# chihyaoma/cyclical-visual-captioning

Hardware: AMD Instinct MI355X
Metric: caption decode-steps/sec (BxT) at N=100,D=2048 (higher is better)
Workload: dtype f32; 1 GPU; cfg2: greedy caption decode; B_per_gpu=64, N=100, F=480, D=2048, A=1024, E=1024, V=5000, T=20, beam=1, hip_graph=True, parallelism=clips sharded over 1 rank(s), no collective, schedule=embedding-gate table (att-LSTM GEMM over K = 2R + one table row per word)

## Files before the change

### cyclical-visual-captioning_amd/build_hip.py

```python
#!/usr/bin/env python3
from __future__ import annotations

import glob
import os
import subprocess
import sys

HERE = os.path.dirname(os.path.abspath(__file__))
CSRC = os.path.join(HERE, "csrc")
OUT_DIR = os.path.join(HERE, "cvc", "lib")
OUT = os.path.join(OUT_DIR, "libcvc_hip.so")
HIPCC = os.environ.get("HIPCC", "/opt/rocm/bin/hipcc")


EXPERIMENTAL_SOURCES = ("gemm_gsk.hip", "gemm_packed_ks.hip")


def experimental() -> bool:
    return os.environ.get("CVC_EXPERIMENTAL", "0") not in ("", "0")


def sources():
    return [f for f in sorted(glob.glob(os.path.join(CSRC, "*.hip")))
            if experimental() or os.path.basename(f) not in EXPERIMENTAL_SOURCES]


def deps():
    inc = os.path.join(os.path.dirname(HERE), "include")
    return sources() + sorted(glob.glob(os.path.join(CSRC, "*.h"))) + \
        [os.path.join(inc, h) for h in ("cvc_hip.h", "cvc_hip_blocks.h", "cvc_hip_experimental.h")]


def source_hash() -> str:
    import hashlib
    h = hashlib.sha256()
    for f in sorted(deps(), key=os.path.basename):
        h.update(os.path.basename(f).encode() + b"\0")
        h.update(open(f, "rb").read())
    return h.hexdigest()[:16]


STAMP = os.path.join(OUT_DIR, "libcvc_hip.flags")


def extra_flags() -> str:
    return " ".join(os.environ.get("CVC_EXTRA_HIPCC_FLAGS", "").split() + (["-DCVC_EXPERIMENTAL"] if experimental() else []))


def up_to_date() -> bool:
    if not os.path.exists(OUT):
        return False
    built_with = open(STAMP).read().strip() if os.path.exists(STAMP) else ""
    if built_with != extra_flags():
        return False
    t = os.path.getmtime(OUT)
    return all(os.path.getmtime(f) <= t for f in deps())


NO_SCRATCH_KERNELS = {"gemm_nn.hip": ("skinny_gemm_nn_split128_kernel",), "gemm_packed.hip": ("skinny_gemm_packed_kernel",)}


def check_no_scratch(src: str, remarks: str):
    import re
    want = NO_SCRATCH_KERNELS.get(os.path.basename(src), ())
    seen = set()
    for block in remarks.split("remark: Function Name: ")[1:]:
        name = block.split()[0]
        hit = next((k for k in want if k in name), None)
        if hit is None:
            continue
        seen.add(hit)
        vals = {k: int(v) for k, v in re.findall(r"remark:\s+(ScratchSize \[bytes/lane\]|SGPRs Spill|VGPRs Spill): (\d+)", block)}
        bad = {k: v for k, v in vals.items() if v != 0}
        if bad or len(vals) < 3:
            raise RuntimeError(f"{os.path.basename(src)}: kernel {name} must not use scratch or spill (inline-assembly loads in "
                               f"flight): {vals}")
    missing = set(want) - seen
    if missing:
        raise RuntimeError(f"{os.path.basename(src)}: no resource-usage remark for {sorted(missing)} (renamed kernel?)")


def build(force: bool = False, verbose: bool = True) -> str:
    if not force and up_to_date():
        return OUT
    os.makedirs(OUT_DIR, exist_ok=True)
    objs = []
    obj_dir = os.path.join(HERE, "build")
    os.makedirs(obj_dir, exist_ok=True)
    procs = []
    for src in sources():
        obj = os.path.join(obj_dir, os.path.basename(src) + ".o")
        objs.append(obj)
        cmd = [HIPCC, "--offload-arch=gfx950", "-O3", "-std=c++17", "-fPIC", "-fvisibility=hidden", "-Wno-comment", "-c", src, "-o", obj]
        cmd += extra_flags().split()
        checked = os.path.basename(src) in NO_SCRATCH_KERNELS
        if checked:
            cmd.append("-Rpass-analysis=kernel-resource-usage")
        if verbose:
            print(" ".join(cmd), flush=True)
        procs.append((cmd, src, checked, subprocess.Popen(cmd, stderr=subprocess.PIPE if checked else None, text=checked or None)))
    for cmd, src, checked, p in procs:
        err = p.communicate()[1] if checked else None
        if p.wait() != 0:
            if err:
                sys.stderr.write("\n".join(l for l in err.splitlines() if "kernel-resource-usage" not in l)[-8000:] + "\n")
            raise RuntimeError("hipcc failed: " + " ".join(cmd))
        if checked:
            check_no_scratch(src, err)
    objs = [o for o in objs if os.path.exists(o)]
    cmd = [HIPCC, "--offload-arch=gfx950", "-shared", "-fPIC", "-o", OUT] + objs + ["-ldl"]
    if verbose:
        print(" ".join(cmd), flush=True)
    subprocess.check_call(cmd)
    with open(STAMP, "w") as f:
        f.write(extra_flags() + "\n")
    return OUT


if __name__ == "__main__":
    print(build(force="--force" in sys.argv))
```

### cyclical-visual-captioning_amd/csrc/attn_scores.h

```cpp
#pragma once
#include "cvc_common.h"
#ifdef CVC_EXPERIMENTAL
#include "gsk.h"
#endif
#include <stdlib.h>
#include <type_traits>

namespace {

#ifndef CVC_SCORE_ROWS
#define CVC_SCORE_ROWS 32
#endif
constexpr int ROWS_PER_WG = CVC_SCORE_ROWS;
constexpr int ROWS_PER_WG_MAX = 128;
constexpr int SCORE_WG = 256;

struct ScoreArgs {
    cvc_attn_set set[2];
    int chunks0;
    const float* q;
    const float* q_bias;
    int q_nparts;
    long long q_part_stride;
    long long q_ld;
    const float* w_a;
    const float* b_a;
    float inv_temp;
    int nq, A;
    int nq_total, q0;
    int rows_per_wg;
#ifdef CVC_EXPERIMENTAL
    int q_from_slab;
    GskSegs q_slab;
#endif
};

template <int NPL>
__device__ __forceinline__ f32x4 sum_planes_fixed(const float* src, long long stride) {
    f32x4 pv[NPL];
#pragma unroll
    for (int p = 0; p < NPL; ++p) pv[p] = ld4(src + (size_t)p * stride);
    f32x4 v = pv[0];
#pragma unroll
    for (int p = 1; p < NPL; ++p) v += pv[p];
    return v;
}
__device__ __forceinline__ f32x4 sum_planes(const float* src, int n, long long stride) {
    switch (n) {
        case 1: return ld4(src);
        case 2: return sum_planes_fixed<2>(src, stride);
        case 4: return sum_planes_fixed<4>(src, stride);
        case 8: return sum_planes_fixed<8>(src, stride);
        case 16: return sum_planes_fixed<16>(src, stride);
        default: break;
    }
    f32x4 v = ld4(src);
    for (int p = 1; p < n; ++p) v += ld4(src + (size_t)p * stride);
    return v;
}

template <int KIND, int NCH, int QG>
__global__ __launch_bounds__(SCORE_WG) void attn_scores_kernel(ScoreArgs a) {
    constexpr bool FACTORABLE = KIND == CVC_ATTN_ADDITIVE && QG > 1;
    extern __shared__ __attribute__((aligned(16))) float smem[];
    const int nq_pad = (a.nq + QG - 1) / QG * QG;
    float* q_s = smem;
    float* w_s = smem + (size_t)nq_pad * a.A;
    constexpr float EXP_C = 2.8853900817779268f;
    const int clip = blockIdx.y;
    const int s = (int)blockIdx.x < a.chunks0 ? 0 : 1;
    const int chunk = s == 0 ? blockIdx.x : blockIdx.x - a.chunks0;
    const cvc_attn_set& S = a.set[s];
    const int A = a.A, nq = a.nq, n = S.n;
    const int tid = threadIdx.x, lane = tid & 63, wave = tid >> 6;
    const float fill = (S.stream & 4) ? -__builtin_inff() : CVC_MIN_VALUE;
    const float bias_a = (KIND == CVC_ATTN_ADDITIVE && a.b_a != nullptr) ? a.b_a[0] : 0.f;

    int q_big = 0;
    for (int i = tid * 4; i < nq_pad * A; i += SCORE_WG * 4) {
        f32x4 v = {0, 0, 0, 0};
#ifdef CVC_EXPERIMENTAL
        if (i < nq * A && a.q_from_slab) {
            const int col = i % A, row = clip * a.nq_total + a.q0 + i / A, blk = col >> 5;
            const int nseg = gsk_nseg(a.q_slab, blk >> 3);
            const float* src = gsk_part(a.q_slab, blk >> 3, 0, blk & 7) + (size_t)row * 32 + (col & 31);
            v = ld4(src);
            for (int p = 1; p < nseg; ++p) v += ld4(src + (size_t)p * (8 * 2048));
            if (a.q_bias != nullptr) v += ld4(a.q_bias + col);
        } else
#endif
        if (i < nq * A) {
            const float* src = a.q + ((size_t)clip * a.nq_total + a.q0 + i / A) * a.q_ld + i % A;
            v = sum_planes(src, a.q_nparts, a.q_part_stride);
            if (a.q_bias != nullptr) v += ld4(a.q_bias + (i % A));
        }
        if (KIND == CVC_ATTN_ADDITIVE) v *= EXP_C;
        if constexpr (FACTORABLE)
            q_big |= !(fabsf(v.x) <= 30.f && fabsf(v.y) <= 30.f && fabsf(v.z) <= 30.f && fabsf(v.w) <= 30.f);
        st4(q_s + i, v);
    }
    if (KIND == CVC_ATTN_ADDITIVE)
        for (int i = tid * 4; i < A; i += SCORE_WG * 4) st4(w_s + i, ld4(a.w_a + i));
    bool factored = false;
    if constexpr (FACTORABLE) {
#ifndef CVC_SCORE_NO_FACTORED
        factored = __syncthreads_or(q_big) == 0;
#else
        __syncthreads();
#endif
        if (factored) {
            for (int i = tid * 4; i < nq_pad * A; i += SCORE_WG * 4) {
                f32x4 v = ld4(q_s + i);
                v.x = __builtin_amdgcn_exp2f(v.x); v.y = __builtin_amdgcn_exp2f(v.y);
                v.z = __builtin_amdgcn_exp2f(v.z); v.w = __builtin_amdgcn_exp2f(v.w);
                st4(q_s + i, v);
            }
            for (int i = tid * 4; i < A; i += SCORE_WG * 4) st4(w_s + i, ld4(w_s + i) * -2.0f);
            __syncthreads();
        }
    } else {
        __syncthreads();
    }

    const int row0 = chunk * a.rows_per_wg;
    const int row_end = min(n, row0 + a.rows_per_wg);
    const float* P = S.proj + (size_t)clip * n * A;

    auto emit = [&](float sc, int q0, int r, bool masked) __attribute__((always_inline)) {
        if (lane < QG && q0 + lane < nq) {
            if (masked) sc = fill;
            const size_t o = ((size_t)clip * a.nq_total + a.q0 + q0 + lane) * n + r;
            S.scores[o] = sc;
            if (S.frame_masked != nullptr)
                S.frame_masked[o] = S.frame_mask[o] != 0 ? fill : sc;
        }
    };
    auto rows = [&](auto stream_tag, auto fact_tag, auto exact_tag) __attribute__((always_inline)) {
        constexpr bool STREAM = decltype(stream_tag)::value;
        constexpr bool FACT = decltype(fact_tag)::value;
        constexpr bool EXACT = decltype(exact_tag)::value;
        const int A = EXACT ? NCH * 256 : a.A;
#define LDF(ptr) (STREAM ? __builtin_nontemporal_load(reinterpret_cast<const f32x4*>(ptr)) : ld4(ptr))
    f32x4 cur[NCH], nxt[NCH];
    int colc[NCH];
    bool cok[NCH];
#pragma unroll
    for (int j = 0; j < NCH; ++j) {
        const int col = (j * 64 + lane) * 4;
        cok[j] = EXACT || col < A;
        colc[j] = cok[j] ? col : A - 4;
    }
    int r = row0 + wave;
    if (r >= row_end) return;
    unsigned mbits = 0;
    if (S.mask != nullptr) {
        const int rr = r + 4 * lane;
        const bool m = rr < row_end && S.mask[(size_t)clip * n + (rr < row_end ? rr : r)] != 0;
        mbits = (unsigned)__builtin_amdgcn_ballot_w64(m);
    }
    float w_total = 0.f;
    if constexpr (FACT) {
#pragma unroll
        for (int j = 0; j < NCH; ++j) {
            const f32x4 w4 = ld4(w_s + colc[j]);
            if (cok[j]) w_total += (w4.x + w4.y) + (w4.z + w4.w);
        }
        w_total = -0.5f * wave_sum(w_total);
    }
#pragma unroll
    for (int j = 0; j < NCH; ++j) cur[j] = LDF(P + (size_t)r * A + colc[j]);
    auto step = [&](f32x4 (&cur)[NCH], f32x4 (&nxt)[NCH], int r, int k) __attribute__((always_inline)) {
#if defined(CVC_SC_ABL) && CVC_SC_ABL == 2
        const int rn = r;
#else
        const int rn = min(r + 4, row_end - 1);
#endif
#pragma unroll
        for (int j = 0; j < NCH; ++j) nxt[j] = LDF(P + (size_t)rn * A + colc[j]);
        const bool masked = (mbits >> k) & 1u;
        if constexpr (FACT) {
            using f32x2 = __attribute__((ext_vector_type(2))) float;
            f32x4 ep[NCH], w2[NCH];
#pragma unroll
            for (int j = 0; j < NCH; ++j) {
                const f32x4 x = cur[j] * EXP_C;
                ep[j].x = __builtin_amdgcn_exp2f(__builtin_amdgcn_fmed3f(x.x, -62.f, 62.f));
                ep[j].y = __builtin_amdgcn_exp2f(__builtin_amdgcn_fmed3f(x.y, -62.f, 62.f));
                ep[j].z = __builtin_amdgcn_exp2f(__builtin_amdgcn_fmed3f(x.z, -62.f, 62.f));
                ep[j].w = __builtin_amdgcn_exp2f(__builtin_amdgcn_fmed3f(x.w, -62.f, 62.f));
                w2[j] = cok[j] ? ld4(w_s + colc[j]) : f32x4{0, 0, 0, 0};
            }
            for (int q0 = 0; q0 < nq; q0 += QG) {
                f32x2 acc2[QG];
                float acc[QG];
#pragma unroll
                for (int u = 0; u < QG; ++u) acc2[u] = f32x2{0.f, 0.f};
#pragma unroll
                for (int j = 0; j < NCH; ++j) {
#pragma unroll
                    for (int u = 0; u < QG; ++u) {
                        const f32x4 eq = ld4(q_s + (q0 + u) * A + colc[j]);
                        const f32x2 d01 = __builtin_elementwise_fma(f32x2{ep[j].x, ep[j].y}, f32x2{eq.x, eq.y}, f32x2{1.0f, 1.0f});
                        const f32x2 d23 = __builtin_elementwise_fma(f32x2{ep[j].z, ep[j].w}, f32x2{eq.z, eq.w}, f32x2{1.0f, 1.0f});
                        const f32x2 r01 = {fast_rcp(d01.x), fast_rcp(d01.y)}, r23 = {fast_rcp(d23.x), fast_rcp(d23.y)};
                        acc2[u] = __builtin_elementwise_fma(f32x2{w2[j].x, w2[j].y}, r01, acc2[u]);
                        acc2[u] = __builtin_elementwise_fma(f32x2{w2[j].z, w2[j].w}, r23, acc2[u]);
                    }
                }
#pragma unroll
                for (int u = 0; u < QG; ++u) acc[u] = (w_total + wave_sum(acc2[u].x + acc2[u].y)) + bias_a;
                float sc = acc[0];
#pragma unroll
                for (int u = 1; u < QG; ++u) sc = lane == u ? acc[u] : sc;
                emit(sc, q0, r, masked);
            }
        } else
        for (int q0 = 0; q0 < nq; q0 += QG) {
            float acc[QG];
            using f32x2 = __attribute__((ext_vector_type(2))) float;
            f32x2 acc2[QG];
#pragma unroll
            for (int u = 0; u < QG; ++u) { acc[u] = 0.f; acc2[u] = f32x2{0.f, 0.f}; }
#pragma unroll
            for (int j = 0; j < NCH; ++j) {
                f32x4 p = cok[j] ? cur[j] : f32x4{0, 0, 0, 0};
                f32x4 w4 = {0, 0, 0, 0};
                if (KIND == CVC_ATTN_ADDITIVE) {
                    w4 = ld4(w_s + colc[j]);
                    if (!cok[j]) w4 = f32x4{0, 0, 0, 0};
                    p *= EXP_C;
                }
#pragma unroll
                for (int u = 0; u < QG; ++u) {
                    const f32x4 q4 = ld4(q_s + (q0 + u) * A + colc[j]);
                    if (KIND == CVC_ATTN_ADDITIVE) {
                        const f32x4 x = p + q4;
                        if constexpr (QG > 1) {
                            const f32x2 e01 = {__builtin_amdgcn_exp2f(x.x), __builtin_amdgcn_exp2f(x.y)};
                            const f32x2 e23 = {__builtin_amdgcn_exp2f(x.z), __builtin_amdgcn_exp2f(x.w)};
                            const f32x2 d01 = e01 + 1.0f, d23 = e23 + 1.0f;
                            const f32x2 r01 = {fast_rcp(d01.x), fast_rcp(d01.y)}, r23 = {fast_rcp(d23.x), fast_rcp(d23.y)};
                            const f32x2 t01 = __builtin_elementwise_fma(f32x2{-2.0f, -2.0f}, r01, f32x2{1.0f, 1.0f});
                            const f32x2 t23 = __builtin_elementwise_fma(f32x2{-2.0f, -2.0f}, r23, f32x2{1.0f, 1.0f});
                            acc2[u] = __builtin_elementwise_fma(f32x2{w4.x, w4.y}, t01, acc2[u]);
                            acc2[u] = __builtin_elementwise_fma(f32x2{w4.z, w4.w}, t23, acc2[u]);
                        } else {
                            acc[u] = fmaf(w4.x, fmaf(-2.0f, fast_rcp(1.0f + __builtin_amdgcn_exp2f(x.x)), 1.0f), acc[u]);
                            acc[u] = fmaf(w4.y, fmaf(-2.0f, fast_rcp(1.0f + __builtin_amdgcn_exp2f(x.y)), 1.0f), acc[u]);
                            acc[u] = fmaf(w4.z, fmaf(-2.0f, fast_rcp(1.0f + __builtin_amdgcn_exp2f(x.z)), 1.0f), acc[u]);
                            acc[u] = fmaf(w4.w, fmaf(-2.0f, fast_rcp(1.0f + __builtin_amdgcn_exp2f(x.w)), 1.0f), acc[u]);
                        }
                    } else {
                        acc[u] += p.x * q4.x + p.y * q4.y + p.z * q4.z + p.w * q4.w;
                    }
                }
            }
            if constexpr (KIND == CVC_ATTN_ADDITIVE && QG > 1) {
#pragma unroll
                for (int u = 0; u < QG; ++u) acc[u] = acc2[u].x + acc2[u].y;
            }
#pragma unroll
            for (int u = 0; u < QG; ++u) acc[u] = KIND == CVC_ATTN_ADDITIVE ? wave_sum(acc[u]) + bias_a : wave_sum(acc[u]) * a.inv_temp;
            float sc = acc[0];
#pragma unroll
            for (int u = 1; u < QG; ++u) sc = lane == u ? acc[u] : sc;
            emit(sc, q0, r, masked);
        }
    };
    for (int k = 0;;) {
        step(cur, nxt, r, k);
        r += 4; ++k;
        if (r >= row_end) break;
        step(nxt, cur, r, k);
        r += 4; ++k;
        if (r >= row_end) break;
    }
#undef LDF
    };
    using T_ = std::true_type;
    using F_ = std::false_type;
    if constexpr (FACTORABLE) {
        if (factored) {
            if (a.A == NCH * 256) { if (S.stream & 1) rows(T_{}, T_{}, T_{}); else rows(F_{}, T_{}, T_{}); }
            else { if (S.stream & 1) rows(T_{}, T_{}, F_{}); else rows(F_{}, T_{}, F_{}); }
            return;
        }
    }
    if (S.stream & 1) rows(T_{}, F_{}, F_{}); else rows(F_{}, F_{}, F_{});
}

template <int KIND, int QG>
int launch_scores_q(const ScoreArgs& a, dim3 grid, size_t lds, hipStream_t st) {
    const int nch = (a.A + 255) / 256;
#define CVC_SC(N) hipLaunchKernelGGL((attn_scores_kernel<KIND, N, QG>), grid, dim3(SCORE_WG), lds, st, a)
    if (nch <= 1) CVC_SC(1);
    else if (nch <= 2) CVC_SC(2);
    else if (nch <= 4) CVC_SC(4);
    else if (nch <= 8) CVC_SC(8);
    else if (nch <= 16) CVC_SC(16);
    else return CVC_E_TOOBIG;
#undef CVC_SC
    return cvc_launch_status();
}

inline int score_group(int nq) {
    if (nq <= 1) return 1;
    const int p4 = (nq + 3) / 4 * 4, p5 = (nq + 4) / 5 * 5;
    return p5 <= p4 ? 5 : 4;
}

template <int KIND>
int launch_scores(const ScoreArgs& a, dim3 grid, size_t lds, hipStream_t st) {
    switch (score_group(a.nq)) {
        case 1: return launch_scores_q<KIND, 1>(a, grid, lds, st);
        case 4: return launch_scores_q<KIND, 4>(a, grid, lds, st);
        default: return launch_scores_q<KIND, 5>(a, grid, lds, st);
    }
}


inline int score_rows_per_wg(int nclip, int n0, int n1, size_t lds_bytes) {
    static const int forced = [] { const char* e = getenv("CVC_SCORE_ROWS_RT"); return e ? atoi(e) : 0; }();
    if (forced >= 4 && forced <= ROWS_PER_WG_MAX) return forced;
    int per_cu = (int)((160 * 1024) / (lds_bytes > 0 ? lds_bytes : 1));
    per_cu = per_cu > 4 ? 4 : (per_cu < 1 ? 1 : per_cu);
    const long long slots = 256LL * per_cu;
    int best = ROWS_PER_WG;
    double best_cost = 1e30;
    for (int r = 8; r <= ROWS_PER_WG_MAX; ++r) {
        const long long wgs = (long long)nclip * ((n0 + r - 1) / r + (n1 > 0 ? (n1 + r - 1) / r : 0));
        const long long rounds = (wgs + slots - 1) / slots;
        const double cost = (double)rounds * ((r + 3) / 4 + 1.5);
        if (cost < best_cost - 1e-9) { best_cost = cost; best = r; }
    }
    return best;
}

inline int run_scores(int kind, const float* q, const float* w_a, const float* b_a, float inv_temp,
                      const cvc_attn_set* sets, int nsets, int nclip, int nq, int A, hipStream_t st,
                      int q_nparts = 1, const float* q_bias = nullptr, const void* q_slab = nullptr, long long q_ld = 0,
                      long long q_part_stride = 0) {
    int q_per_launch = (int)((64 * 1024) / ((size_t)A * 4)) - 1;
    if (q_per_launch < 1) return CVC_E_TOOBIG;
    if (q_per_launch > nq) q_per_launch = nq;
    if (q_per_launch < nq && q_per_launch >= 5) q_per_launch = q_per_launch / 5 * 5;
    while (q_per_launch > 1 && (size_t)((q_per_launch + score_group(q_per_launch) - 1) / score_group(q_per_launch) *
                                        score_group(q_per_launch) + 1) * A * 4 > 64 * 1024) --q_per_launch;
    ScoreArgs sa;
    sa.set[0] = sets[0];
    sa.set[1] = nsets > 1 ? sets[1] : sets[0];
    sa.q = q; sa.w_a = w_a; sa.b_a = b_a; sa.inv_temp = inv_temp; sa.A = A; sa.nq_total = nq;
    sa.q_nparts = q_nparts < 1 ? 1 : q_nparts; sa.q_bias = q_bias;
    sa.q_ld = q_ld > 0 ? q_ld : A;
    sa.q_part_stride = q_part_stride > 0 ? q_part_stride : (long long)nclip * nq * A;
#ifdef CVC_EXPERIMENTAL
    sa.q_from_slab = q_slab != nullptr;
    sa.q_slab = q_slab != nullptr ? *static_cast<const GskSegs*>(q_slab) : GskSegs{};
#else
    if (q_slab != nullptr) return CVC_E_BADARG;
#endif
    for (int q0 = 0; q0 < nq; q0 += q_per_launch) {
        sa.q0 = q0;
        sa.nq = nq - q0 < q_per_launch ? nq - q0 : q_per_launch;
        const int qg = score_group(sa.nq);
        const size_t lds1 = (size_t)((sa.nq + qg - 1) / qg * qg + 1) * A * sizeof(float);
        sa.rows_per_wg = sa.nq > 1 ? score_rows_per_wg(nclip, sets[0].n, nsets > 1 ? sets[1].n : 0, lds1) : ROWS_PER_WG;
        sa.chunks0 = (sets[0].n + sa.rows_per_wg - 1) / sa.rows_per_wg;
        const int chunks1 = nsets > 1 ? (sets[1].n + sa.rows_per_wg - 1) / sa.rows_per_wg : 0;
        dim3 g1(sa.chunks0 + chunks1, nclip);
        int rc = kind == CVC_ATTN_ADDITIVE ? launch_scores<CVC_ATTN_ADDITIVE>(sa, g1, lds1, st)
                                           : launch_scores<CVC_ATTN_DOT>(sa, g1, lds1, st);
        if (rc != 0) return rc;
    }
    return 0;
}

}
```

Baseline: 330,800 decode-steps/s.

## Balance single-query attention score work across CUs with row shares and prefetch

For the single-query (decode) path, the score kernel now splits the combined rows of both attention sets into evenly sized shares whose count is chosen from the CU count and clip count, so one workgroup may span both sets. Each wave prefetches its first projection row and mask before the query-plane summation, the 16-plane query sum is split into two batches of loads, and launch bounds request higher occupancy for small-NCH QG=1 variants. The build adds a scratch/spill check for those kernels. This aims to cut tail imbalance and load latency in the per-step attention, at the cost of more register pressure and extra code paths.

```diff
diff --git a/cyclical-visual-captioning_amd/build_hip.py b/cyclical-visual-captioning_amd/build_hip.py
--- a/cyclical-visual-captioning_amd/build_hip.py
+++ b/cyclical-visual-captioning_amd/build_hip.py
@@ -57,7 +57,8 @@
     return all(os.path.getmtime(f) <= t for f in deps())
 
 
-NO_SCRATCH_KERNELS = {"gemm_nn.hip": ("skinny_gemm_nn_split128_kernel",), "gemm_packed.hip": ("skinny_gemm_packed_kernel",)}
+NO_SCRATCH_KERNELS = {"gemm_nn.hip": ("skinny_gemm_nn_split128_kernel",), "gemm_packed.hip": ("skinny_gemm_packed_kernel",),
+                      "attn_fwd.hip": ("attn_scores_kernelILi0ELi4ELi1E", "attn_scores_kernelILi1ELi4ELi1E")}
 
 
 def check_no_scratch(src: str, remarks: str):
diff --git a/cyclical-visual-captioning_amd/csrc/attn_scores.h b/cyclical-visual-captioning_amd/csrc/attn_scores.h
--- a/cyclical-visual-captioning_amd/csrc/attn_scores.h
+++ b/cyclical-visual-captioning_amd/csrc/attn_scores.h
@@ -29,6 +29,8 @@
     int nq, A;
     int nq_total, q0;
     int rows_per_wg;
+    int shares;
+    int rows_total;
 #ifdef CVC_EXPERIMENTAL
     int q_from_slab;
     GskSegs q_slab;
@@ -59,8 +61,10 @@
     return v;
 }
 
+constexpr int score_min_waves(int nch, int qg) { return qg == 1 && nch <= 4 ? 5 : 1; }
+
 template <int KIND, int NCH, int QG>
-__global__ __launch_bounds__(SCORE_WG) void attn_scores_kernel(ScoreArgs a) {
+__global__ __launch_bounds__(SCORE_WG, score_min_waves(NCH, QG)) void attn_scores_kernel(ScoreArgs a) {
     constexpr bool FACTORABLE = KIND == CVC_ATTN_ADDITIVE && QG > 1;
     extern __shared__ __attribute__((aligned(16))) float smem[];
     const int nq_pad = (a.nq + QG - 1) / QG * QG;
@@ -68,13 +72,53 @@
     float* w_s = smem + (size_t)nq_pad * a.A;
     constexpr float EXP_C = 2.8853900817779268f;
     const int clip = blockIdx.y;
-    const int s = (int)blockIdx.x < a.chunks0 ? 0 : 1;
-    const int chunk = s == 0 ? blockIdx.x : blockIdx.x - a.chunks0;
-    const cvc_attn_set& S = a.set[s];
-    const int A = a.A, nq = a.nq, n = S.n;
+    const int A = a.A, nq = a.nq;
     const int tid = threadIdx.x, lane = tid & 63, wave = tid >> 6;
-    const float fill = (S.stream & 4) ? -__builtin_inff() : CVC_MIN_VALUE;
+    int part_set[2], part_lo[2], part_hi[2], nparts = 1;
+    if (QG == 1 && a.shares > 0) {
+        const int n0 = a.set[0].n;
+        const int lo = (int)((long long)blockIdx.x * a.rows_total / a.shares);
+        const int hi = (int)((long long)(blockIdx.x + 1) * a.rows_total / a.shares);
+        if (lo < n0) {
+            part_set[0] = 0; part_lo[0] = lo; part_hi[0] = min(hi, n0);
+            part_set[1] = 1; part_lo[1] = 0; part_hi[1] = hi - n0;
+            nparts = hi > n0 ? 2 : 1;
+        } else {
+            part_set[0] = 1; part_lo[0] = lo - n0; part_hi[0] = hi - n0;
+            part_set[1] = 1; part_lo[1] = 0; part_hi[1] = 0;
+        }
+    } else {
+        const int s = (int)blockIdx.x < a.chunks0 ? 0 : 1;
+        const int chunk = s == 0 ? blockIdx.x : blockIdx.x - a.chunks0;
+        part_set[0] = s; part_lo[0] = chunk * a.rows_per_wg; part_hi[0] = min(a.set[s].n, part_lo[0] + a.rows_per_wg);
+        part_set[1] = s; part_lo[1] = 0; part_hi[1] = 0;
+    }
     const float bias_a = (KIND == CVC_ATTN_ADDITIVE && a.b_a != nullptr) ? a.b_a[0] : 0.f;
+
+    using T_ = std::true_type;
+    using F_ = std::false_type;
+    auto run = [&](auto pre_tag) __attribute__((always_inline)) {
+    constexpr bool PRE_NT = decltype(pre_tag)::value;
+    f32x4 pre[NCH];
+    int pre_mask = 0;
+    if constexpr (QG == 1) {
+        const cvc_attn_set& S = a.set[part_set[0]];
+        const int n = S.n;
+        const int r = min(part_lo[0] + wave, n - 1);
+        const float* src = S.proj + ((size_t)clip * n + r) * A;
+        if constexpr (PRE_NT) asm volatile("" ::: "memory");
+#pragma unroll
+        for (int j = 0; j < NCH; ++j) {
+            const int col = (j * 64 + lane) * 4;
+            const f32x4* p4 = reinterpret_cast<const f32x4*>(src + (col < A ? col : A - 4));
+            pre[j] = PRE_NT ? __builtin_nontemporal_load(p4) : *p4;
+        }
+        if constexpr (PRE_NT) asm volatile("" ::: "memory");
+        if (S.mask != nullptr) {
+            const int rr = part_lo[0] + wave + 4 * lane;
+            pre_mask = S.mask[(size_t)clip * n + (rr < part_hi[0] ? rr : r)];
+        }
+    }
 
     int q_big = 0;
     for (int i = tid * 4; i < nq_pad * A; i += SCORE_WG * 4) {
@@ -91,7 +135,17 @@
 #endif
         if (i < nq * A) {
             const float* src = a.q + ((size_t)clip * a.nq_total + a.q0 + i / A) * a.q_ld + i % A;
-            v = sum_planes(src, a.q_nparts, a.q_part_stride);
+            if (QG == 1 && a.q_nparts == 16) {
+                v = sum_planes_fixed<8>(src, a.q_part_stride);
+                asm volatile("" : "+v"(v) :: "memory");
+                f32x4 pv[8];
+#pragma unroll
+                for (int p = 0; p < 8; ++p) pv[p] = ld4(src + (size_t)(8 + p) * a.q_part_stride);
+#pragma unroll
+                for (int p = 0; p < 8; ++p) v += pv[p];
+            } else {
+                v = sum_planes(src, a.q_nparts, a.q_part_stride);
+            }
             if (a.q_bias != nullptr) v += ld4(a.q_bias + (i % A));
         }
         if (KIND == CVC_ATTN_ADDITIVE) v *= EXP_C;
@@ -122,8 +176,14 @@
         __syncthreads();
     }
 
-    const int row0 = chunk * a.rows_per_wg;
-    const int row_end = min(n, row0 + a.rows_per_wg);
+    if constexpr (QG == 1) {
+        asm volatile("" : "+v"(pre_mask));
+    }
+    auto part = [&](const int s, const int row0, const int row_end, auto first_tag) __attribute__((always_inline)) {
+    constexpr bool FIRST = QG == 1 && decltype(first_tag)::value;
+    const cvc_attn_set& S = a.set[s];
+    const int n = S.n;
+    const float fill = (S.stream & 4) ? -__builtin_inff() : CVC_MIN_VALUE;
     const float* P = S.proj + (size_t)clip * n * A;
 
     auto emit = [&](float sc, int q0, int r, bool masked) __attribute__((always_inline)) {
@@ -155,7 +215,10 @@
     unsigned mbits = 0;
     if (S.mask != nullptr) {
         const int rr = r + 4 * lane;
-        const bool m = rr < row_end && S.mask[(size_t)clip * n + (rr < row_end ? rr : r)] != 0;
+        int mb;
+        if (FIRST) mb = pre_mask;
+        else mb = S.mask[(size_t)clip * n + (rr < row_end ? rr : r)];
+        const bool m = rr < row_end && mb != 0;
         mbits = (unsigned)__builtin_amdgcn_ballot_w64(m);
     }
     float w_total = 0.f;
@@ -167,8 +230,13 @@
         }
         w_total = -0.5f * wave_sum(w_total);
     }
-#pragma unroll
-    for (int j = 0; j < NCH; ++j) cur[j] = LDF(P + (size_t)r * A + colc[j]);
+    if (FIRST) {
+#pragma unroll
+        for (int j = 0; j < NCH; ++j) cur[j] = pre[j];
+    } else {
+#pragma unroll
+        for (int j = 0; j < NCH; ++j) cur[j] = LDF(P + (size_t)r * A + colc[j]);
+    }
     auto step = [&](f32x4 (&cur)[NCH], f32x4 (&nxt)[NCH], int r, int k) __attribute__((always_inline)) {
 #if defined(CVC_SC_ABL) && CVC_SC_ABL == 2
         const int rn = r;
@@ -277,8 +345,10 @@
     }
 #undef LDF
     };
-    using T_ = std::true_type;
-    using F_ = std::false_type;
+    if constexpr (FIRST) {
+        rows(pre_tag, F_{}, F_{});
+        return;
+    }
     if constexpr (FACTORABLE) {
         if (factored) {
             if (a.A == NCH * 256) { if (S.stream & 1) rows(T_{}, T_{}, T_{}); else rows(F_{}, T_{}, T_{}); }
@@ -287,6 +357,17 @@
         }
     }
     if (S.stream & 1) rows(T_{}, F_{}, F_{}); else rows(F_{}, F_{}, F_{});
+    };
+    part(part_set[0], part_lo[0], part_hi[0], T_{});
+    if constexpr (QG == 1) {
+        if (nparts > 1) part(part_set[1], part_lo[1], part_hi[1], F_{});
+    }
+    };
+    if constexpr (QG == 1) {
+        if (a.set[part_set[0]].stream & 1) run(T_{}); else run(F_{});
+    } else {
+        run(F_{});
+    }
 }
 
 template <int KIND, int QG>
@@ -332,6 +413,31 @@
         const long long rounds = (wgs + slots - 1) / slots;
         const double cost = (double)rounds * ((r + 3) / 4 + 1.5);
         if (cost < best_cost - 1e-9) { best_cost = cost; best = r; }
+    }
+    return best;
+}
+
+constexpr int SCORE_SHARE_ROWS = 36;
+inline int score_shares(int nclip, int rows_total) {
+    static const int forced = [] { const char* e = getenv("CVC_SCORE_SHARES_RT"); return e ? atoi(e) : 0; }();
+    static const int ncu = [] {
+        int dev = 0, n = 0;
+        if (hipGetDevice(&dev) != hipSuccess || hipDeviceGetAttribute(&n, hipDeviceAttributeMultiprocessorCount, dev) != hipSuccess) n = 0;
+        return n;
+    }();
+    const int w_min = (rows_total + ROWS_PER_WG_MAX - 1) / ROWS_PER_WG_MAX;
+    if (forced < 0) return 0;
+    if (forced > 0) return forced >= w_min && forced <= 65535 ? forced : 0;
+    if (ncu < 1) return 0;
+    int g = ncu, b = nclip;
+    while (b != 0) { const int t = g % b; g = b; b = t; }
+    const int unit = ncu / g;
+    int best = 0;
+    long long best_d = 0;
+    for (int w = unit; w <= rows_total && w <= 65535; w += unit) {
+        if (w < w_min) continue;
+        const long long d = llabs((long long)rows_total - (long long)w * SCORE_SHARE_ROWS);
+        if (best == 0 || d * best < best_d * w) { best = w; best_d = d; }
     }
     return best;
 }
@@ -367,7 +473,9 @@
         sa.rows_per_wg = sa.nq > 1 ? score_rows_per_wg(nclip, sets[0].n, nsets > 1 ? sets[1].n : 0, lds1) : ROWS_PER_WG;
         sa.chunks0 = (sets[0].n + sa.rows_per_wg - 1) / sa.rows_per_wg;
         const int chunks1 = nsets > 1 ? (sets[1].n + sa.rows_per_wg - 1) / sa.rows_per_wg : 0;
-        dim3 g1(sa.chunks0 + chunks1, nclip);
+        sa.rows_total = sets[0].n + (nsets > 1 ? sets[1].n : 0);
+        sa.shares = sa.nq == 1 ? score_shares(nclip, sa.rows_total) : 0;
+        dim3 g1(sa.shares > 0 ? sa.shares : sa.chunks0 + chunks1, nclip);
         int rc = kind == CVC_ATTN_ADDITIVE ? launch_scores<CVC_ATTN_ADDITIVE>(sa, g1, lds1, st)
                                            : launch_scores<CVC_ATTN_DOT>(sa, g1, lds1, st);
         if (rc != 0) return rc;
```

Result: no change. 330,000 decode-steps/s (-0.2%).
